# izhengfan/se2lam

Hardware: NVIDIA H100
Metric: ORB keypoints/sec at 640x480 (8-level pyramid, 1000 kps/frame) (higher is better)
Workload: dtype u8

## Files before the change

se2lam_b200/csrc/fast_screen.h:

```cpp
#pragma once
#include <cstdint>

#if defined(__CUDACC__)
#define SE2_HD __host__ __device__ __forceinline__
#else
#define SE2_HD inline
#endif

namespace fastpx {
SE2_HD int16_t lo16(unsigned a) { return (int16_t)(a & 0xFFFF); }
SE2_HD int16_t hi16(unsigned a) { return (int16_t)(a >> 16); }
SE2_HD unsigned pack16(int lo, int hi) { return ((unsigned)lo & 0xFFFFu) | ((unsigned)hi << 16); }
SE2_HD unsigned perm(unsigned a, unsigned b, unsigned s) {
#if defined(__CUDA_ARCH__)
    return __byte_perm(a, b, s);
#else
    const uint64_t src = ((uint64_t)b << 32) | a;
    unsigned r = 0;
    for (int i = 0; i < 4; ++i) {
        const unsigned sel = (s >> (4 * i)) & 0xF;
        unsigned byte = (unsigned)(src >> (8 * (sel & 7))) & 0xFF;
        if (sel & 8) byte = (byte & 0x80) ? 0xFF : 0x00;
        r |= byte << (8 * i);
    }
// ... 38 lines not shown
}

namespace fastpx {

SE2_HD unsigned screen_bias(int t) { return (unsigned)(511 - t) * 0x10001u; }

SE2_HD unsigned screen4(unsigned n3, unsigned s3, unsigned n2l, unsigned n2c, unsigned n2r, unsigned s2l, unsigned s2c, unsigned s2r,
                        unsigned zl, unsigned zc, unsigned zr, unsigned bias) {
    const unsigned w_m3 = perm(zl, zc, 0x4321), w_p3 = perm(zc, zr, 0x6543);
    const unsigned nw_ = perm(n2l, n2c, 0x5432), ne_ = perm(n2c, n2r, 0x5432);
    const unsigned sw_ = perm(s2l, s2c, 0x5432), se_ = perm(s2c, s2r, 0x5432);
    unsigned ok[2];
#if defined(__CUDA_ARCH__)
#pragma unroll
#endif
    for (int hlf = 0; hlf < 2; ++hlf) {
        const unsigned sel = hlf ? 0x4341u : 0x4240u;
        const unsigned v = perm(zc, 0, sel);
        const unsigned p0 = perm(s3, 0, sel), p8 = perm(n3, 0, sel);
        const unsigned p4 = perm(w_p3, 0, sel), p12 = perm(w_m3, 0, sel);
        const unsigned p2 = perm(se_, 0, sel), p10 = perm(nw_, 0, sel);
        const unsigned p6 = perm(ne_, 0, sel), p14 = perm(sw_, 0, sel);
        const unsigned lo = maxs2(max3s2(mins2(p0, p8), mins2(p4, p12), mins2(p2, p10)), mins2(p6, p14));
        const unsigned hi = mins2(min3s2(maxs2(p0, p8), maxs2(p4, p12), maxs2(p2, p10)), maxs2(p6, p14));
        ok[hlf] = ((v + bias - lo) | (hi + bias - v)) & 0x02000200u;
    }
    const unsigned b = ok[0] + (ok[1] << 1);
    return ((b >> 9) | (b >> 23)) & 0xFu;
}
SE2_HD unsigned screen_T1(int t) { return screen_bias(t); }
SE2_HD unsigned screen_U1(int t) { return screen_bias(t); }
SE2_HD unsigned screen4(unsigned n3, unsigned s3, unsigned n2l, unsigned n2c, unsigned n2r, unsigned s2l, unsigned s2c, unsigned s2r,
                        unsigned zl, unsigned zc, unsigned zr, unsigned T1, unsigned ) {
    return screen4(n3, s3, n2l, n2c, n2r, s2l, s2c, s2r, zl, zc, zr, T1);
}

SE2_HD unsigned inside_mask8(int x0, int cw) {
    const int lo = x0 < 0 ? -x0 : 0;
    const int hi = cw - x0 < 8 ? cw - x0 : 8;
    return (0xFFu << lo) & (0xFFu >> (8 - hi)) & 0xFFu;
}

SE2_HD int first_group(int shift) { return (shift + 3) >> 2; }
SE2_HD int groups_per_row(int cw, int shift) { return ((shift + 2 + cw) >> 2) - first_group(shift) + 1; }
SE2_HD int group_x0(int g, int shift) { return 4 * (g + first_group(shift)) - 3 - shift; }
SE2_HD int items_per_row(int cw, int shift) { return (groups_per_row(cw, shift) + 1) >> 1; }
struct ItemWalk {
    int y, g, dY, dG, G;
    SE2_HD void init(int tid, int nthreads, int groups) { G = groups; y = tid / G; g = tid - y * G; dY = nthreads / G; dG = nthreads - dY * G; }
    SE2_HD void next() { g += dG; y += dY; if (g >= G) { g -= G; ++y; } }
};

constexpr int NMS_X0 = 4;
SE2_HD int nms_plane_bytes(int pw, int ch) { return pw * (ch + 2) + 32; }
SE2_HD int nms_words_per_row(int cw) { return (cw + 31) >> 5; }
SE2_HD unsigned nms_row_mask(int k, int cw) { const int n = cw - 32 * k; return n >= 32 ? 0xFFFFFFFFu : (1u << n) - 1u; }

SE2_HD unsigned nms32(const uint32_t* u, const uint32_t* c, const uint32_t* d) {
    unsigned c3e[10], c3o[10];
    unsigned r[4];
#if defined(__CUDA_ARCH__)
#pragma unroll
#endif
    for (int j = 0; j < 10; ++j) {
        const unsigned ua = u[j], ca = c[j], da = d[j];
        if (j > 0) c3e[j] = max3s2(perm(ua, 0, 0x4240), perm(ca, 0, 0x4240), perm(da, 0, 0x4240));
        if (j < 9) c3o[j] = max3s2(perm(ua, 0, 0x4341), perm(ca, 0, 0x4341), perm(da, 0, 0x4341));
    }
#if defined(__CUDA_ARCH__)
#pragma unroll
#endif
    for (int g = 0; g < 8; ++g) {
        const int j = g + 1;
        const unsigned ua = u[j], ca = c[j], da = d[j];
        const unsigned ce = perm(ca, 0, 0x4240), co = perm(ca, 0, 0x4341);
        const unsigned ve = maxs2(perm(ua, 0, 0x4240), perm(da, 0, 0x4240));
        const unsigned vo = maxs2(perm(ua, 0, 0x4341), perm(da, 0, 0x4341));
        const unsigned ne = max3s2(perm(c3o[j - 1], c3o[j], 0x5432), ve, c3o[j]);
        const unsigned no = max3s2(c3e[j], vo, perm(c3e[j], c3e[j + 1], 0x5432));
        const unsigned te = ce + 0x00FF00FFu - ne, to = co + 0x00FF00FFu - no;
        const unsigned bytes = perm(te, to, 0x7351);
        if (g & 1) {
            r[g >> 1] = (r[g >> 1] + (bytes << 4)) * 0x01020408u;
        } else {
            r[g >> 1] = bytes;
        }
    }
    return perm(perm(r[0], r[1], 0x7373), perm(r[2], r[3], 0x7373), 0x5410);
}

struct WordRun {
    int w, w1, y, k, wpr;
    SE2_HD void init(int tid, int nthreads, int ch, int words_per_row) {
        wpr = words_per_row;
        const int nw = ch * wpr, q = (nw + nthreads - 1) / nthreads;
        w = tid * q < nw ? tid * q : nw;
        w1 = w + q < nw ? w + q : nw;
        y = w / wpr; k = w - y * wpr;
    }
    SE2_HD bool more() const { return w < w1; }
    SE2_HD void next() { ++w; if (++k == wpr) { k = 0; ++y; } }
};

}
```

se2lam_b200/csrc/orb.cu:

```cuda
#include <cuda.h>

#include <algorithm>
#include <cmath>
#include <cstring>
#include <type_traits>
#include <vector>

#include "blur_px.h"
#include "common.h"
#include "fast_screen.h"
#include "introselect.h"
#include "resp_key.h"

namespace {

using se2gpu::fail;

constexpr int EDGE = 16;
constexpr int HALF_PATCH = 15;
constexpr int PATCH = 31;
constexpr int MAX_LEVELS = 16;
constexpr int FAST_THREADS = 256;
constexpr int ORB_LANES = 4;
constexpr int BLUR_WARPS = 4;
// ... 247 lines not shown
            for (int r = ty; r < nsr; r += 8) {
                const uint8_t* rp = raw + r * raw_pitch;
                const unsigned h0 = (unsigned)((rp[sx0[0]] * a0[0] + rp[sx1[0]] * a1[0]) >> 4), h1 = (unsigned)((rp[sx0[1]] * a0[1] + rp[sx1[1]] * a1[1]) >> 4);
                const unsigned h2 = (unsigned)((rp[sx0[2]] * a0[2] + rp[sx1[2]] * a1[2]) >> 4), h3 = (unsigned)((rp[sx0[3]] * a0[3] + rp[sx1[3]] * a1[3]) >> 4);
                *reinterpret_cast<uint2*>(hbuf + r * 128 + 4 * tx) = make_uint2((h0 & 0xFFFFu) | (h1 << 16), (h2 & 0xFFFFu) | (h3 << 16));
            }
        }
    }
    __syncthreads();
    if (x4 >= L.pitch) return;
    uint8_t* plane = d.plain + f * d.frame_plane_bytes + L.plane_off;
#pragma unroll
    for (int k = 0; k < RESIZE_TR / 8; ++k) {
        const int r = ty + 8 * k, y = y0 + r;
        if (y >= H) break;
        uint32_t word = 0;
        if (x4 < W) {
            const ResizeRow ri = rowinfo[r];
            const uint2 A = *reinterpret_cast<const uint2*>(hbuf + (ri.s0 - r_lo) * 128 + 4 * tx);
            const uint2 B = *reinterpret_cast<const uint2*>(hbuf + (ri.s1 - r_lo) * 128 + 4 * tx);
            const unsigned v0 = (unsigned)((((ri.b0 * (int)(A.x & 0xFFFFu)) >> 16) + ((ri.b1 * (int)(B.x & 0xFFFFu)) >> 16) + 2) >> 2);
            const unsigned v1 = (unsigned)((((ri.b0 * (int)(A.x >> 16)) >> 16) + ((ri.b1 * (int)(B.x >> 16)) >> 16) + 2) >> 2);
            const unsigned v2 = (unsigned)((((ri.b0 * (int)(A.y & 0xFFFFu)) >> 16) + ((ri.b1 * (int)(B.y & 0xFFFFu)) >> 16) + 2) >> 2);
            const unsigned v3 = (unsigned)((((ri.b0 * (int)(A.y >> 16)) >> 16) + ((ri.b1 * (int)(B.y >> 16)) >> 16) + 2) >> 2);
            word = (v0 | (v1 << 8) | (v2 << 16) | (v3 << 24)) & vmask;
        }
        *reinterpret_cast<uint32_t*>(plane + (size_t)y * L.pitch + x4) = word;
    }
}

__device__ __forceinline__ unsigned fast_cv(int v) { return (unsigned)(256 + v) | ((unsigned)(256 - v) << 16); }
__device__ __forceinline__ unsigned fast_q(unsigned p, unsigned cv) { return p * 0xFFFFu + cv; }

__device__ __forceinline__ int fast_arc_score(const uint8_t* __restrict__ p, int pw) {
    const unsigned cv = fast_cv(p[0]);
    unsigned q[16];
    q[0] = fast_q(p[3 * pw], cv);       q[1] = fast_q(p[3 * pw + 1], cv);   q[2] = fast_q(p[2 * pw + 2], cv);    q[3] = fast_q(p[pw + 3], cv);
    q[4] = fast_q(p[3], cv);            q[5] = fast_q(p[-pw + 3], cv);      q[6] = fast_q(p[-2 * pw + 2], cv);   q[7] = fast_q(p[-3 * pw + 1], cv);
    q[8] = fast_q(p[-3 * pw], cv);      q[9] = fast_q(p[-3 * pw - 1], cv);  q[10] = fast_q(p[-2 * pw - 2], cv);  q[11] = fast_q(p[-pw - 3], cv);
    q[12] = fast_q(p[-3], cv);          q[13] = fast_q(p[pw - 3], cv);      q[14] = fast_q(p[2 * pw - 2], cv);   q[15] = fast_q(p[3 * pw - 1], cv);
    unsigned m3[16];
#pragma unroll
    for (int k = 0; k < 16; ++k) m3[k] = __vimin3_s16x2(q[k], q[(k + 1) & 15], q[(k + 2) & 15]);
    unsigned best = 0;
#pragma unroll
    for (int k = 0; k < 16; k += 2) {
        const unsigned a9 = __vimin3_s16x2(m3[k], m3[(k + 3) & 15], m3[(k + 6) & 15]);
        const unsigned b9 = __vimin3_s16x2(m3[k + 1], m3[(k + 4) & 15], m3[(k + 7) & 15]);
        best = __vimax3_s16x2(best, a9, b9);
    }
    return (int)max(best & 0xFFFFu, best >> 16) - 256;
}

struct FastMaps { CUtensorMap m[MAX_LEVELS]; };
__device__ __forceinline__ unsigned orb_smem_u32(const void* p) { return (unsigned)__cvta_generic_to_shared(p); }
__device__ __forceinline__ void orb_mbar_init(unsigned long long* bar, unsigned count) {
    asm volatile("mbarrier.init.shared::cta.b64 [%0], %1;" ::"r"(orb_smem_u32(bar)), "r"(count) : "memory");
    asm volatile("fence.mbarrier_init.release.cluster;" ::: "memory");
}
__device__ __forceinline__ bool orb_mbar_wait(unsigned long long* bar, unsigned parity) {
    const long long t0 = clock64();
    for (;;) {
        unsigned done;
        asm volatile(
            "{\n"
            ".reg .pred p;\n"
            "mbarrier.try_wait.parity.shared::cta.b64 p, [%1], %2;\n"
            "selp.u32 %0, 1, 0, p;\n"
            "}\n" : "=r"(done) : "r"(orb_smem_u32(bar)), "r"(parity) : "memory");
        if (done) return true;
        if (clock64() - t0 > 400000000LL) return false;
    }
}
__device__ __forceinline__ void orb_tma_box3(void* dst_smem, const CUtensorMap* map, int x, int y, int z, unsigned bytes, unsigned long long* bar) {
    asm volatile("mbarrier.arrive.expect_tx.shared::cta.b64 _, [%0], %1;" ::"r"(orb_smem_u32(bar)), "r"(bytes) : "memory");
    asm volatile("cp.async.bulk.tensor.3d.shared::cluster.global.tile.mbarrier::complete_tx::bytes [%0], [%1, {%2, %3, %4}], [%5];"
                 ::"r"(orb_smem_u32(dst_smem)), "l"(map), "r"(x), "r"(y), "r"(z), "r"(orb_smem_u32(bar)) : "memory");
}

template <bool TMA>
__global__ void __launch_bounds__(FAST_THREADS, 5) orb_fast_cells(OrbDev d, const __grid_constant__ FastMaps maps) {
    extern __shared__ __align__(128) uint8_t smem_raw[];
    __shared__ int s_ncand, s_wsum[FAST_THREADS / 32];
    __shared__ __align__(8) unsigned long long s_bar;
    const CellGeo c = d.cells[blockIdx.x];
    const int f = blockIdx.y + d.frame0;
    CellHdr* hdr = d.hdr + (size_t)f * d.n_cells + blockIdx.x;
    const int cw = c.x1 - c.x0, ch = c.y1 - c.y0;
    if (c.skipped || cw <= 0 || ch <= 0) {
        if (threadIdx.x == 0) { hdr->n_base = 0; hdr->n_a = 0; hdr->n_b = 0; }
        return;
    }
    const LevelGeo& L = d.levels[c.level];
    const int bx0 = c.x0 - 3 + EDGE, ax0 = bx0 & (TMA ? ~15 : ~3), shift = bx0 - ax0;
    const int pw = TMA ? L.fbw : (shift + cw + 6 + 3) & ~3, pww = pw >> 2;
    const int ph = TMA ? L.fbh : ch + 6;
    uint8_t* smem = TMA ? smem_raw + ((128u - (orb_smem_u32(smem_raw) & 127u)) & 127u) : smem_raw;
    const int g0 = fastpx::first_group(shift), G = fastpx::items_per_row(cw, shift), nitems = ch * G;
    const int wpr = fastpx::nms_words_per_row(cw);
    uint8_t* patch = smem;
    uint8_t* score = smem + ((pw * ph + 15) & ~15);
    uint32_t* bitmap = reinterpret_cast<uint32_t*>(score + ((fastpx::nms_plane_bytes(pw, ch) + 15) & ~15));
    uint16_t* list = reinterpret_cast<uint16_t*>(bitmap + ch * wpr);
    if (TMA) {
        if (threadIdx.x == 0) orb_mbar_init(&s_bar, 1);
        __syncthreads();
        if (threadIdx.x == 0) orb_tma_box3(patch, &maps.m[c.level], ax0, c.y0 - 3 + EDGE, f, (unsigned)(pw * ph), &s_bar);
    } else {
        const uint8_t* plane = d.plain + f * d.frame_plane_bytes + L.plane_off;
        const int by0 = c.y0 - 3 + EDGE;
        for (int i = threadIdx.x; i < pww * ph; i += FAST_THREADS) {
            const int py = i / pww, pxw = i - py * pww;
            reinterpret_cast<uint32_t*>(patch)[i] = *reinterpret_cast<const uint32_t*>(plane + (size_t)(by0 + py) * L.pitch + ax0 + 4 * pxw);
        }
    }
    constexpr int NW = FAST_THREADS / 32;
    const int lane = threadIdx.x & 31, wid = threadIdx.x >> 5;
    const uint8_t* p0 = patch + 3 * pw + 3 + shift;
    fastpx::ItemWalk first;
    first.init((int)threadIdx.x, FAST_THREADS, G);
    fastpx::WordRun words;
    words.init((int)threadIdx.x, FAST_THREADS, ch, wpr);
    int thr = d.fast_th;
    int total = 0, pos0 = 0;
    for (int pass = 0; pass < 2; ++pass) {
        for (int i = threadIdx.x; i < pw * (ch + 2) / 4; i += FAST_THREADS) reinterpret_cast<uint32_t*>(score)[i] = 0u;
        if (threadIdx.x == 0) s_ncand = 0;
        if (TMA && pass == 0 && !orb_mbar_wait(&s_bar, 0)) { *d.err = 4; return; }
        __syncthreads();
        {
            const uint32_t* pwords = reinterpret_cast<const uint32_t*>(patch);
            const unsigned bias = fastpx::screen_bias(thr);
            fastpx::ItemWalk it = first;
            for (int it0 = wid * 32; it0 < nitems; it0 += NW * 32) {
                unsigned m = 0;
                const int col0 = fastpx::group_x0(2 * it.g, shift);
                if (it.y < ch) {
                    const uint32_t* c = pwords + (it.y + 3) * pww + 2 * it.g + g0;
                    const uint32_t n3a = c[-3 * pww], n3b = c[-3 * pww + 1], s3a = c[3 * pww], s3b = c[3 * pww + 1];
                    const uint32_t n2a = c[-2 * pww - 1], n2b = c[-2 * pww], n2c = c[-2 * pww + 1], n2d = c[-2 * pww + 2];
                    const uint32_t s2a = c[2 * pww - 1], s2b = c[2 * pww], s2c = c[2 * pww + 1], s2d = c[2 * pww + 2];
                    const uint32_t za = c[-1], zb = c[0], zc = c[1], zd = c[2];
                    m = (fastpx::screen4(n3a, s3a, n2a, n2b, n2c, s2a, s2b, s2c, za, zb, zc, bias) |
                         fastpx::screen4(n3b, s3b, n2b, n2c, n2d, s2b, s2c, s2d, zb, zc, zd, bias) << 4) & fastpx::inside_mask8(col0, cw);
                }
                uint16_t* dst = list + atomicAdd(&s_ncand, __popc(m));
                const int e0 = it.y * pw + col0;
#pragma unroll
                for (int j = 0; j < 8; ++j)
                    if (m & (1u << j)) *dst++ = (uint16_t)(e0 + j);
                it.next();
            }
        }
        __syncthreads();
        const int ncand = s_ncand;
        for (int i = threadIdx.x; i < ncand; i += FAST_THREADS) {
            const int off = list[i];
            const int m = fast_arc_score(p0 + off, pw);
            if (m > thr) score[off + pw + fastpx::NMS_X0] = (uint8_t)(m - 1);
        }
        __syncthreads();
        int nkp = 0;
        for (fastpx::WordRun r = words; r.more(); r.next()) {
            const uint32_t* u = reinterpret_cast<const uint32_t*>(score) + r.y * pww + 8 * r.k;
            const unsigned bits = fastpx::nms32(u, u + pww, u + 2 * pww) & fastpx::nms_row_mask(r.k, cw);
            bitmap[r.w] = bits;
            nkp += __popc(bits);
        }
        int inc = nkp;
#pragma unroll
        for (int o = 1; o < 32; o <<= 1) { const int u = __shfl_up_sync(0xffffffffu, inc, o); if (lane >= o) inc += u; }
        if (lane == 31) s_wsum[wid] = inc;
        __syncthreads();
        total = 0; pos0 = inc - nkp;
#pragma unroll
        for (int w = 0; w < NW; ++w) { const int v = s_wsum[w]; total += v; if (w < wid) pos0 += v; }
        if (total > 3 || thr == 7) break;
        thr = 7;
    }
    uint32_t* out = d.cand + (size_t)f * d.cand_total + c.cand_off;
    int pos = pos0;
    for (fastpx::WordRun r = words; r.more(); r.next()) {
        uint32_t bits = bitmap[r.w];
        const uint8_t* srow = score + (r.y + 1) * pw + fastpx::NMS_X0 + 32 * r.k;
        const uint32_t yx = ((uint32_t)(c.y0 + r.y) << 12) | (uint32_t)(c.x0 + 32 * r.k);
        while (bits) {
            const int i = __ffs(bits) - 1;
            bits &= bits - 1;
            if (pos < c.cand_cap) out[pos] = ((uint32_t)srow[i] << 24) | (yx + i);
            else *d.err = 1;
            ++pos;
        }
    }
    if (threadIdx.x == 0) { hdr->n_base = total; hdr->n_a = total; hdr->n_b = total; }
}

__device__ __forceinline__ int fast_arc_score_qr(const uint8_t* __restrict__ p, int pw, int t) {
    const int v = p[0];
    const int c0 = v - p[3 * pw], c8 = v - p[-3 * pw];
    bool dk = (c0 > t) | (c8 > t), br = (c0 < -t) | (c8 < -t);
    if (!(dk | br)) return 0;
    const int c4 = v - p[3], c12 = v - p[-3];
    dk &= (c4 > t) | (c12 > t); br &= (c4 < -t) | (c12 < -t);
    if (!(dk | br)) return 0;
    const int c2 = v - p[2 * pw + 2], c10 = v - p[-2 * pw - 2];
    dk &= (c2 > t) | (c10 > t); br &= (c2 < -t) | (c10 < -t);
    if (!(dk | br)) return 0;
    const int c6 = v - p[-2 * pw + 2], c14 = v - p[2 * pw - 2];
    dk &= (c6 > t) | (c14 > t); br &= (c6 < -t) | (c14 < -t);
    if (!(dk | br)) return 0;
#define SE2_PK(dv) ((static_cast<unsigned>(dv) & 0xFFFFu) | (static_cast<unsigned>(-(dv)) << 16))
    unsigned q[16];
    q[0] = SE2_PK(c0);   q[1] = SE2_PK(v - p[3 * pw + 1]);    q[2] = SE2_PK(c2);    q[3] = SE2_PK(v - p[pw + 3]);
    q[4] = SE2_PK(c4);   q[5] = SE2_PK(v - p[-pw + 3]);       q[6] = SE2_PK(c6);    q[7] = SE2_PK(v - p[-3 * pw + 1]);
    q[8] = SE2_PK(c8);   q[9] = SE2_PK(v - p[-3 * pw - 1]);   q[10] = SE2_PK(c10);  q[11] = SE2_PK(v - p[-pw - 3]);
    q[12] = SE2_PK(c12); q[13] = SE2_PK(v - p[pw - 3]);       q[14] = SE2_PK(c14);  q[15] = SE2_PK(v - p[3 * pw - 1]);
#undef SE2_PK
    unsigned m3[16];
#pragma unroll
    for (int k = 0; k < 16; ++k) m3[k] = __vimin3_s16x2(q[k], q[(k + 1) & 15], q[(k + 2) & 15]);
    unsigned best = 0x80008000u;
#pragma unroll
    for (int k = 0; k < 16; k += 2) {
        const unsigned a9 = __vimin3_s16x2(m3[k], m3[(k + 3) & 15], m3[(k + 6) & 15]);
        const unsigned b9 = __vimin3_s16x2(m3[k + 1], m3[(k + 4) & 15], m3[(k + 7) & 15]);
        best = __vimax3_s16x2(best, a9, b9);
    }
    const int mdark = static_cast<short>(best & 0xFFFFu), mbright = static_cast<short>(best >> 16);
    return max(mdark, mbright);
}

__global__ void __launch_bounds__(FAST_THREADS) orb_fast_cells_big(OrbDev d) {
    extern __shared__ uint8_t smem[];
    __shared__ int s_total;
    const CellGeo c = d.cells[blockIdx.x];
    const int f = blockIdx.y + d.frame0;
    CellHdr* hdr = d.hdr + (size_t)f * d.n_cells + blockIdx.x;
    const int cw = c.x1 - c.x0, ch = c.y1 - c.y0;
    if (c.skipped || cw <= 0 || ch <= 0) {
        if (threadIdx.x == 0) { hdr->n_base = 0; hdr->n_a = 0; hdr->n_b = 0; }
        return;
    }
    const LevelGeo& L = d.levels[c.level];
    const uint8_t* plane = d.plain + f * d.frame_plane_bytes + L.plane_off;
    const int bx0 = c.x0 - 3 + EDGE, by0 = c.y0 - 3 + EDGE;
    const int ax0 = bx0 & ~3, shift = bx0 - ax0;
    const int ph = ch + 6, sw = cw + 2, sh = ch + 2;
// ... 486 lines not shown
    int kp_off = 0;
    const float imageRatio = (float)w / (float)hgt;
    for (int l = 0; l < nl; ++l) {
        LevelGeo& g = L[l];
        const float scale = h->mvInvScaleFactor[l];
        g.w = cv_round_f((float)w * scale); g.h = cv_round_f((float)hgt * scale);
        if (g.w < 2 * EDGE + 7 || g.h < 2 * EDGE + 7) return fail(SE2GPU_ERR_INVALID, "level %d of a %dx%d frame is %dx%d: too small for the 16 px border", l, w, hgt, g.w, g.h);
        if (g.w + 2 * EDGE > 4095 || g.h + 2 * EDGE > 4095) return fail(SE2GPU_ERR_CAPACITY, "frames wider/taller than 4063 px are not supported");
        g.pitch = (g.w + 2 * EDGE + 31) & ~31;
        g.plane_off = poff;
        poff += (size_t)g.pitch * (g.h + 2 * EDGE);
        poff = (poff + 255) & ~(size_t)255;
        g.nDesired = h->mnFeaturesPerLevel[l];
        g.cols = (int)sqrtf((float)g.nDesired / (5 * imageRatio));
        g.rows = (int)(imageRatio * g.cols);
        if (g.cols < 1 || g.rows < 1) return fail(SE2GPU_ERR_INVALID, "level %d has a %dx%d cell grid (nfeatures too small): undefined in the reference", l, g.cols, g.rows);
        const int minB = EDGE, maxBX = g.w - EDGE, maxBY = g.h - EDGE;
        const int W = maxBX - minB, H = maxBY - minB;
        const int cellW = (int)ceilf((float)W / g.cols), cellH = (int)ceilf((float)H / g.rows);
        g.nCells = g.rows * g.cols;
        g.nfeaturesCell = (int)ceilf((float)g.nDesired / g.nCells);
        g.cell_base = (int)C.size();
        g.kp_off = kp_off; g.kp_cap = g.nDesired; kp_off += g.nDesired;
        g.scale = h->mvScaleFactor[l];
        g.kp_size = (float)(int)(PATCH * h->mvScaleFactor[l]);
        g.tab_off = (int)toff; toff += (size_t)g.w + g.h;
        std::vector<int> iniXCol(g.cols, 0);
        const size_t first_cell = C.size();
        int max_cw = 0, max_ch = 0;
        float hY = cellH + 6;
        for (int i = 0; i < g.rows; ++i) {
            const float iniY = minB + i * cellH - 3;
            bool rowSkipped = false;
            if (i == g.rows - 1) { hY = maxBY + 3 - iniY; if (hY <= 0) rowSkipped = true; }
            float hX = cellW + 6;
            for (int j = 0; j < g.cols; ++j) {
                CellGeo c{};
                c.level = l;
                if (rowSkipped) { c.skipped = 1; C.push_back(c); continue; }
                float iniX;
                if (i == 0) { iniX = minB + j * cellW - 3; iniXCol[j] = (int)iniX; } else iniX = iniXCol[j];
                if (j == g.cols - 1) { hX = maxBX + 3 - iniX; if (hX <= 0) { c.skipped = 1; C.push_back(c); continue; } }
                const int r0 = (int)iniY, r1 = (int)(iniY + hY), c0 = (int)iniX, c1 = (int)(iniX + hX);
                if (r1 > g.h || c1 > g.w || r0 < 0 || c0 < 0) return fail(SE2GPU_ERR_INVALID, "cell grid of level %d leaves the image (the reference asserts here)", l);
                c.x0 = c0 + 3; c.x1 = c1 - 3; c.y0 = r0 + 3; c.y1 = r1 - 3;
                const int cw = std::max(c.x1 - c.x0, 0), chh = std::max(c.y1 - c.y0, 0);
                c.cand_off = (int)coff;
                c.cand_cap = ((cw + 1) / 2) * ((chh + 1) / 2) + 8;
                coff += c.cand_cap;
                if (cw > 0 && chh > 0) {
                    max_cw = std::max(max_cw, ((c.x0 - 3 + EDGE) & 15) + cw); max_ch = std::max(max_ch, chh);
                    const size_t pwb = (size_t)((cw + 6 + 3 + 3) / 4 + 1) * 4;
                    const size_t bitmap = (size_t)chh * fastpx::nms_words_per_row(cw) * 4;
                    if (pwb * (chh + 6) > 65535) fast_big = true;
                    fsm = std::max(fsm, ((pwb * (chh + 6) + 15) & ~(size_t)15) + (((size_t)fastpx::nms_plane_bytes((int)pwb, chh) + 15) & ~(size_t)15) + bitmap + (size_t)cw * chh * 2 + 64);
                    const size_t nchunk = (size_t)chh * ((cw + 31) / 32);
                    fsm_big = std::max(fsm_big, ((pwb * (chh + 6) + 15) & ~(size_t)15) + (((size_t)(cw + 2) * (chh + 2) + 15) & ~(size_t)15) + nchunk * 4 + 64);
                }
                C.push_back(c);
            }
        }
        g.fbw = (max_cw + 6 + 15) & ~15; g.fbh = max_ch + 6;
        if (max_cw > 0) {
            if (g.fbw > 256 || g.fbh > 256 || (size_t)g.fbw * g.fbh > 65535) tma_ok = false;
            for (size_t ci = first_cell; ci < C.size(); ++ci) {
                const int cw = C[ci].x1 - C[ci].x0, chh = C[ci].y1 - C[ci].y0;
                if (C[ci].skipped || cw <= 0 || chh <= 0) continue;
                const size_t pw = (size_t)g.fbw, bitmap = (size_t)chh * fastpx::nms_words_per_row(cw) * 4;
                fsm_tma = std::max(fsm_tma, (size_t)128 + ((pw * g.fbh + 15) & ~(size_t)15) + (((size_t)fastpx::nms_plane_bytes(g.fbw, chh) + 15) & ~(size_t)15) + bitmap + (size_t)cw * chh * 2 + 64);
            }
        }
        if (h->harris) ssm = std::max(ssm, (size_t)(2 * g.nDesired + 4 * g.nCells + 64) * 8 + (size_t)g.nCells * 16 + (size_t)(SEL_STAGE / 2) * 8);
        else ssm = std::max(ssm, (size_t)(2 * g.nDesired + 4 * g.nCells + 64) * 4 + (size_t)g.nCells * 16 + (size_t)SEL_STAGE * 4);
        g.tile_base = (int)T.size();
        g.blur_strips = std::max(2, (g.h + BLUR_TH - 1) / BLUR_TH);
        g.blur_th = ((g.h + g.blur_strips - 1) / g.blur_strips + 12) / 7 * 7 - 6;
        for (int it = 0; it < g.blur_strips * (g.pitch / 8); it += 32) T.push_back(TileGeo{l, it / (g.pitch / 8), it % (g.pitch / 8)});
    }
    *plane_bytes = poff; *cand_total = coff; *n_cells = C.size(); *n_tiles = T.size(); *tab_total = toff;
    if (fsm > 227 * 1024) fast_big = true;
    *max_fast_smem = fast_big ? fsm_big : fsm; *max_select_smem = ssm;
    if (fast_big_out) *fast_big_out = fast_big;
    if (fast_tma_smem_out) *fast_tma_smem_out = (tma_ok && !fast_big && fsm_tma <= 227 * 1024) ? fsm_tma : 0;
    if (Lv) *Lv = L;
    if (Cv) *Cv = C;
    if (Tv) *Tv = T;
    return SE2GPU_OK;
}

typedef CUresult (*EncodeTiledFn)(CUtensorMap*, CUtensorMapDataType, cuuint32_t, void*, const cuuint64_t*, const cuuint64_t*, const cuuint32_t*,
                                  const cuuint32_t*, CUtensorMapInterleave, CUtensorMapSwizzle, CUtensorMapL2promotion, CUtensorMapFloatOOBfill);
EncodeTiledFn tensor_map_encoder() {
    static EncodeTiledFn fn = [] {
        void* p = nullptr;
        cudaDriverEntryPointQueryResult q = cudaDriverEntryPointSymbolNotFound;
        if (cudaGetDriverEntryPoint("cuTensorMapEncodeTiled", &p, cudaEnableDefault, &q) != cudaSuccess || q != cudaDriverEntryPointSuccess) { cudaGetLastError(); p = nullptr; }
        return (EncodeTiledFn)p;
    }();
    return fn;
}

constexpr int BLUR_SPLIT = 1;
constexpr int PIPE_CHUNKS = 4, PIPE_FIRST_PCT = 50, SUBMIT_CHUNKS = 1;

bool encode_fast_maps(se2gpu_orb* h, size_t frame_plane_bytes) {
    EncodeTiledFn enc = tensor_map_encoder();
    if (!enc || (frame_plane_bytes & 15)) return false;
    for (int l = 0; l < h->nlevels; ++l) {
        const LevelGeo& g = h->levels[l];
        if (g.fbw <= 6) { memset(&h->fast_maps.m[l], 0, sizeof(CUtensorMap)); continue; }
        const cuuint64_t gdim[3] = {(cuuint64_t)g.pitch, (cuuint64_t)(g.h + 2 * EDGE), (cuuint64_t)h->max_batch};
        const cuuint64_t gstr[2] = {(cuuint64_t)g.pitch, (cuuint64_t)frame_plane_bytes};
        const cuuint32_t box[3] = {(cuuint32_t)g.fbw, (cuuint32_t)g.fbh, 1u};
        const cuuint32_t estr[3] = {1u, 1u, 1u};
        void* base = h->d.plain + g.plane_off;
        if (((uintptr_t)base & 15) || (g.pitch & 15)) return false;
        if (enc(&h->fast_maps.m[l], CU_TENSOR_MAP_DATA_TYPE_UINT8, 3, base, gdim, gstr, box, estr, CU_TENSOR_MAP_INTERLEAVE_NONE,
                CU_TENSOR_MAP_SWIZZLE_NONE, CU_TENSOR_MAP_L2_PROMOTION_L2_128B, CU_TENSOR_MAP_FLOAT_OOB_FILL_NONE) != CUDA_SUCCESS) return false;
    }
    return true;
}

int set_geometry(se2gpu_orb* h, int w, int hgt, cudaStream_t s) {
    if (w == h->cur_w && hgt == h->cur_h) return SE2GPU_OK;
    size_t pb, ct, nc, nt, tt, fsm, ssm, fsm_tma = 0;
    bool big = false;
    int rc = build_geometry(h, w, hgt, false, &pb, &ct, &nc, &nt, &tt, &fsm, &ssm, &h->levels, &h->cells, &h->tiles, &big, &fsm_tma);
    if (rc != SE2GPU_OK) return rc;
    if (pb > h->cap_plane || ct > h->cap_cand || nc > h->cap_cells || nt > h->cap_tiles || tt > h->cap_tab)
        return fail(SE2GPU_ERR_CAPACITY, "frame %dx%d exceeds the capacity this extractor was created with (%dx%d)", w, hgt, h->max_w, h->max_h);
    if (fsm > 227 * 1024) return fail(SE2GPU_ERR_CAPACITY, "a FAST cell of a %dx%d frame needs %zu B of shared memory", w, hgt, fsm);
    std::vector<int> itab(tt, 0);
    std::vector<short> stab(2 * tt, 0);
    for (int l = 1; l < h->nlevels; ++l) {
        const LevelGeo& g = h->levels[l];
        const LevelGeo& sg = h->levels[l - 1];
        const double scale_x = 1. / ((double)g.w / sg.w), scale_y = 1. / ((double)g.h / sg.h);
        int* xofs = itab.data() + g.tab_off; int* yofs = xofs + g.w;
        short* ialpha = stab.data() + 2 * (size_t)g.tab_off; short* ibeta = ialpha + 2 * g.w;
        for (int dx = 0; dx < g.w; ++dx) {
            float fx = (float)((dx + 0.5) * scale_x - 0.5);
            int sx = (int)floorf(fx);
            fx -= sx;
            if (sx < 0) { fx = 0; sx = 0; }
            if (sx >= sg.w - 1) { fx = 0; sx = sg.w - 1; }
            xofs[dx] = sx;
            ialpha[2 * dx] = (short)std::min(std::max(cv_round_f((1.f - fx) * 2048.f), -32768), 32767);
            ialpha[2 * dx + 1] = (short)std::min(std::max(cv_round_f(fx * 2048.f), -32768), 32767);
        }
        for (int dy = 0; dy < g.h; ++dy) {
            float fy = (float)((dy + 0.5) * scale_y - 0.5);
            int sy = (int)floorf(fy);
            fy -= sy;
            yofs[dy] = sy;
            ibeta[2 * dy] = (short)cv_round_f((1.f - fy) * 2048.f);
            ibeta[2 * dy + 1] = (short)cv_round_f(fy * 2048.f);
        }
    }
    SE2_CUDA(cudaMemcpyAsync(h->d_levels, h->levels.data(), sizeof(LevelGeo) * h->levels.size(), cudaMemcpyHostToDevice, s));
    SE2_CUDA(cudaMemcpyAsync(h->d_cells, h->cells.data(), sizeof(CellGeo) * h->cells.size(), cudaMemcpyHostToDevice, s));
    SE2_CUDA(cudaMemcpyAsync(h->d_tiles, h->tiles.data(), sizeof(TileGeo) * h->tiles.size(), cudaMemcpyHostToDevice, s));
    SE2_CUDA(cudaMemcpyAsync(h->d_itab, itab.data(), sizeof(int) * itab.size(), cudaMemcpyHostToDevice, s));
// ... 117 lines not shown
    d.frame0 = frame0;
    cudaStream_t side = lane < 0 ? h->side : nullptr;
    cudaEvent_t ev_pyr = h->ev_pyr, ev_blur = h->ev_blur;
    se2gpu::Profiler& pr = h->prof;
    SE2_NVTX("se2gpu.orb.run_device");
    nvtxRangePushA("se2gpu.orb.pyramid");
    pr.begin(0, s);
    {
        const LevelGeo& g = h->levels[0];
        if (h->und_on) {
            dim3 grid((g.pitch / 4 + 127) / 128, g.h + 2 * EDGE, n);
            SE2_LAUNCH(orb_pyr0_undistort, grid, 128, 0, s, d, g, d_imgs, stride, frame_stride, h->d_und_m1, h->d_und_m2);
        } else {
            const int aligned = (((uintptr_t)d_imgs | (uintptr_t)stride | (uintptr_t)frame_stride) & 15) == 0;
            const int nvec = aligned ? g.w / 16 : 0;
            dim3 grid((nvec + 63) / 64 + 1, (g.h + 2 * EDGE + 4 * PYR0_ROWS - 1) / (4 * PYR0_ROWS), n);
            SE2_LAUNCH(orb_pyr0, grid, dim3(64, 4), 0, s, d, g, d_imgs, stride, frame_stride, nvec);
        }
    }
    const int splitA = std::min(BLUR_SPLIT, h->nlevels);
    for (int l = 1; l < h->nlevels; ++l) {
        const LevelGeo& g = h->levels[l];
        cudaLaunchConfig_t cfg = {};
        const int ncx = (g.pitch + 127) / 128, H = g.h + 2 * EDGE;
        const int tall_grid = ncx * ((H + RESIZE_TR_TALL - 1) / RESIZE_TR_TALL) * n;
        const bool tall = h->resize_tall_ctas > 0 && tall_grid >= h->resize_tall_ctas;
        const int tr = tall ? RESIZE_TR_TALL : RESIZE_TR;
        cfg.gridDim = dim3(ncx, (H + tr - 1) / tr, n);
        cfg.blockDim = dim3(32, 8); cfg.dynamicSmemBytes = tall ? h->resize_tall_smem : h->resize_w_smem; cfg.stream = s;
        cudaLaunchAttribute at[1];
        at[0].id = cudaLaunchAttributeProgrammaticStreamSerialization;
        at[0].val.programmaticStreamSerializationAllowed = 1;
        cfg.attrs = at; cfg.numAttrs = 1;
        if (tall) SE2_CUDA(cudaLaunchKernelEx(&cfg, orb_resize_w<RESIZE_TR_TALL>, d, g, h->levels[l - 1], h->resize_tall_rows, h->resize_raw_pitch));
        else SE2_CUDA(cudaLaunchKernelEx(&cfg, orb_resize_w<RESIZE_TR>, d, g, h->levels[l - 1], h->resize_rows, h->resize_raw_pitch));
        ::se2gpu::g_launches.fetch_add(1, std::memory_order_relaxed);
        if (l == splitA - 1 && side && !pr.on) SE2_CUDA(cudaEventRecord(h->ev_l1, s));
    }
    if (splitA - 1 <= 0 && side && !pr.on) SE2_CUDA(cudaEventRecord(h->ev_l1, s));
    pr.end(s);
    nvtxRangePop();
    const bool overlap = !pr.on && side != nullptr;
    auto launch_blur = [&](cudaStream_t st, int t0, int t1) {
        if (t1 > t0) SE2_LAUNCH(orb_blur, dim3((t1 - t0 + BLUR_WARPS - 1) / BLUR_WARPS, n), BLUR_WARPS * 32, 0, st, d, t0, t1);
    };
    const int tilesA = splitA < h->nlevels ? h->levels[splitA].tile_base : d.n_tiles;
    if (overlap) {
        SE2_CUDA(cudaStreamWaitEvent(side, h->ev_l1, 0));
        launch_blur(side, 0, tilesA);
    }
    SE2_NVTX("se2gpu.orb.fast_select_blur_describe");
    pr.begin(1, s);
    if (h->fast_big) SE2_LAUNCH(orb_fast_cells_big, dim3(d.n_cells, n), FAST_THREADS, h->fast_smem, s, d);
    else if (h->fast_tma) SE2_LAUNCH(orb_fast_cells<true>, dim3(d.n_cells, n), FAST_THREADS, h->fast_tma_smem, s, d, h->fast_maps);
    else SE2_LAUNCH(orb_fast_cells<false>, dim3(d.n_cells, n), FAST_THREADS, h->fast_smem, s, d, h->fast_maps);
    if (h->harris) SE2_LAUNCH(orb_harris, dim3(d.n_cells, n), HARRIS_THREADS, 0, s, d, h->hb.cand64);
    pr.end(s);
    if (overlap) {
        SE2_CUDA(cudaEventRecord(ev_pyr, s));
        SE2_CUDA(cudaStreamWaitEvent(side, ev_pyr, 0));
        launch_blur(side, tilesA, d.n_tiles);
        SE2_CUDA(cudaEventRecord(ev_blur, side));
    }
    pr.begin(2, s);
    if (h->harris) SE2_LAUNCH(orb_select<true>, dim3(h->nlevels, n), SEL_THREADS, h->select_smem, s, d, h->hb);
    else SE2_LAUNCH(orb_select<false>, dim3(h->nlevels, n), SEL_THREADS, h->select_smem, s, d, h->hb);
    pr.end(s);
    if (overlap) {
        SE2_CUDA(cudaStreamWaitEvent(s, ev_blur, 0));
    } else {
        pr.begin(3, s);
        launch_blur(s, 0, d.n_tiles);
        pr.end(s);
    }
    const int warps = 8;
    pr.begin(4, s);
    if (h->harris) SE2_LAUNCH(orb_orient_describe<true>, dim3((h->nfeatures + warps - 1) / warps, n), warps * 32, 0, s, d, d_kps, d_desc, d_counts, h->hb.lresp);
    else SE2_LAUNCH(orb_orient_describe<false>, dim3((h->nfeatures + warps - 1) / warps, n), warps * 32, 0, s, d, d_kps, d_desc, d_counts, h->hb.lresp);
    pr.end(s);
    h->last_n = std::max(h->last_n * (frame0 > 0), frame0 + n);
    return SE2GPU_OK;
}

}

extern "C" {

se2gpu_orb* se2gpu_orb_create_scored(int nfeatures, float scale_factor, int nlevels, int score_type, int fast_th, int max_w, int max_h,
                                     int max_batch, int device) {
    if (score_type != SE2GPU_ORB_HARRIS_SCORE && score_type != SE2GPU_ORB_FAST_SCORE) {
        fail(SE2GPU_ERR_INVALID, "unknown ORB score type %d (HARRIS_SCORE = 0, FAST_SCORE = 1)", score_type); return nullptr;
    }
    if (nfeatures <= 0 || nlevels <= 0 || nlevels > MAX_LEVELS || !(scale_factor > 1.0f) || fast_th < 1 || fast_th > 254 ||
        max_w <= 0 || max_h <= 0 || max_batch <= 0) { fail(SE2GPU_ERR_INVALID, "bad ORB parameters"); return nullptr; }
    if (se2gpu::select_device(device) != SE2GPU_OK) return nullptr;
    se2gpu_orb* h = new se2gpu_orb;
    h->device = device; h->nfeatures = nfeatures; h->nlevels = nlevels; h->fast_th = fast_th;
    h->harris = score_type == SE2GPU_ORB_HARRIS_SCORE;
    h->max_w = max_w; h->max_h = max_h; h->max_batch = max_batch;
    { int* a = h->create_args; a[0] = nfeatures; memcpy(&a[1], &scale_factor, sizeof(float)); a[2] = nlevels; a[3] = fast_th; a[4] = max_w; a[5] = max_h; a[6] = max_batch; a[7] = device; a[8] = score_type; }
    h->scaleFactor = scale_factor;
    h->mvScaleFactor.resize(nlevels); h->mvInvScaleFactor.resize(nlevels); h->mnFeaturesPerLevel.resize(nlevels);
    h->mvScaleFactor[0] = 1;
    for (int i = 1; i < nlevels; i++) h->mvScaleFactor[i] = (float)(h->mvScaleFactor[i - 1] * h->scaleFactor);
    const float invScaleFactor = (float)(1.0f / h->scaleFactor);
    h->mvInvScaleFactor[0] = 1;
    for (int i = 1; i < nlevels; i++) h->mvInvScaleFactor[i] = h->mvInvScaleFactor[i - 1] * invScaleFactor;
    const float factor = (float)(1.0 / h->scaleFactor);
// ... 243 lines not shown
int se2gpu_orb_set_undistort(se2gpu_orb* h, const float* K, const float* dist, int ndist) {
    if (!h) return fail(SE2GPU_ERR_INVALID, "null handle");
    if (!K) { h->und_on = false; return SE2GPU_OK; }
    if (ndist != 0 && ndist != 4 && ndist != 5 && ndist != 8 && ndist != 12 && ndist != 14) return fail(SE2GPU_ERR_INVALID, "distortion vector must have 0, 4, 5, 8, 12 or 14 coefficients");
    if (ndist > 0 && !dist) return fail(SE2GPU_ERR_INVALID, "null distortion vector");
    if (ndist == 14 && (dist[12] != 0.f || dist[13] != 0.f)) return fail(SE2GPU_ERR_INVALID, "tilted-sensor coefficients (tauX, tauY) are not supported");
    memcpy(h->und_K, K, sizeof h->und_K);
    memset(h->und_D, 0, sizeof h->und_D);
    if (ndist > 0) memcpy(h->und_D, dist, sizeof(float) * ndist);
    h->und_nd = ndist; h->und_w = h->und_h = 0; h->und_on = true;
    return SE2GPU_OK;
}

int se2gpu_orb_debug_undistort_map(const float* K, const float* dist, int ndist, int w, int hgt, int16_t* m1, uint16_t* m2) {
    if (!K || !m1 || !m2 || w <= 0 || hgt <= 0 || ndist < 0 || ndist > 14 || (ndist > 0 && !dist)) return fail(SE2GPU_ERR_INVALID, "bad argument");
    std::vector<short2> a; std::vector<uint16_t> b;
    int rc = build_undistort_map(K, dist, ndist, w, hgt, a, b);
    if (rc != SE2GPU_OK) return rc;
    memcpy(m1, a.data(), a.size() * sizeof(short2));
    memcpy(m2, b.data(), b.size() * sizeof(uint16_t));
    return SE2GPU_OK;
}

int se2gpu_orb_profile(se2gpu_orb* h, int enable) {
    if (!h) return fail(SE2GPU_ERR_INVALID, "null handle");
    SE2_CUDA(cudaSetDevice(h->device));
    h->prof.enable(enable != 0);
    return SE2GPU_OK;
}

int se2gpu_orb_profile_read(se2gpu_orb* h, double* ms, int* launches) {
    if (!h) return fail(SE2GPU_ERR_INVALID, "null handle");
    SE2_CUDA(cudaSetDevice(h->device));
    h->prof.flush();
    for (int g = 0; g < SE2GPU_ORB_PROFILE_GROUPS; ++g) { if (ms) ms[g] = h->prof.ms[g]; if (launches) launches[g] = h->prof.launches[g]; }
    return SE2GPU_OK;
}

int se2gpu_orb_level_dims(se2gpu_orb* h, int level, int* w, int* hgt, int* pitch) {
    if (!h || level < 0 || level >= h->nlevels || h->cur_w < 0) return fail(SE2GPU_ERR_INVALID, "no geometry");
    *w = h->levels[level].w; *hgt = h->levels[level].h; *pitch = h->levels[level].pitch;
    return SE2GPU_OK;
}

int se2gpu_orb_get_level(se2gpu_orb* h, int frame, int level, int blurred, uint8_t* out) {
    if (!h || level < 0 || level >= h->nlevels || h->cur_w < 0 || frame < 0 || frame >= h->last_n) return fail(SE2GPU_ERR_INVALID, "bad frame/level");
    SE2_CUDA(cudaSetDevice(h->device));
    const LevelGeo& g = h->levels[level];
    const uint8_t* src = (blurred ? h->d.blurred : h->d.plain) + (size_t)frame * h->d.frame_plane_bytes + g.plane_off;
    SE2_CUDA(cudaMemcpy(out, src, (size_t)g.pitch * (g.h + 2 * EDGE), cudaMemcpyDeviceToHost));
    return SE2GPU_OK;
}

}
```

Measured before the change: 109.6 million.

## Pad NMS score pitch, flatten FAST grid cell-major, pass box dims in maps

The NMS score plane now uses a separate pitch (pw | 4), which skews rows to reduce shared-memory bank conflicts in the 3-row nms32 reads. The TMA path adds a per-row skew via a reciprocal multiply to map patch offsets to the padded score layout. The FAST launch is flattened to a 1D grid, ordered cell-major with frames interleaved, so blocks for the same cell across frames run adjacently. Box dimensions now come from the grid-constant FastMaps instead of the global level struct. Optional clock instrumentation is added behind a compile flag. The padding uses slightly more shared memory per block, which may affect occupancy.

New measurement: 112.2 million, median of 6. +2.4%, better.

```diff
diff --git a/se2lam_b200/csrc/fast_screen.h b/se2lam_b200/csrc/fast_screen.h
--- a/se2lam_b200/csrc/fast_screen.h
+++ b/se2lam_b200/csrc/fast_screen.h
@@ -114,7 +114,8 @@
 };
 
 constexpr int NMS_X0 = 4;
-SE2_HD int nms_plane_bytes(int pw, int ch) { return pw * (ch + 2) + 32; }
+SE2_HD int nms_pitch(int pw) { return pw | 4; }
+SE2_HD int nms_plane_bytes(int sp, int ch) { return sp * (ch + 2) + 32; }
 SE2_HD int nms_words_per_row(int cw) { return (cw + 31) >> 5; }
 SE2_HD unsigned nms_row_mask(int k, int cw) { const int n = cw - 32 * k; return n >= 32 ? 0xFFFFFFFFu : (1u << n) - 1u; }
 
diff --git a/se2lam_b200/csrc/orb.cu b/se2lam_b200/csrc/orb.cu
--- a/se2lam_b200/csrc/orb.cu
+++ b/se2lam_b200/csrc/orb.cu
@@ -323,7 +323,7 @@
     return (int)max(best & 0xFFFFu, best >> 16) - 256;
 }
 
-struct FastMaps { CUtensorMap m[MAX_LEVELS]; };
+struct FastMaps { CUtensorMap m[MAX_LEVELS]; int fbw[MAX_LEVELS], fbh[MAX_LEVELS]; };
 __device__ __forceinline__ unsigned orb_smem_u32(const void* p) { return (unsigned)__cvta_generic_to_shared(p); }
 __device__ __forceinline__ void orb_mbar_init(unsigned long long* bar, unsigned count) {
     asm volatile("mbarrier.init.shared::cta.b64 [%0], %1;" ::"r"(orb_smem_u32(bar)), "r"(count) : "memory");
@@ -349,34 +349,56 @@
                  ::"r"(orb_smem_u32(dst_smem)), "l"(map), "r"(x), "r"(y), "r"(z), "r"(orb_smem_u32(bar)) : "memory");
 }
 
+#ifdef SE2GPU_FAST_PASS_CLOCKS
+enum FastClk { CLK_ENTRY = 0, CLK_LANDED = 1, CLK_PASS0 = 2,  CLK_END = 8,
+               CLK_INFO = 9 , CLK_GT0 = 10, CLK_GT1 = 11, CLK_ISSUED = 12 ,
+               FAST_CLK_SLOTS = 13 };
+__device__ unsigned long long* g_fast_clk;
+__device__ __forceinline__ unsigned long long orb_globaltimer() { unsigned long long t; asm volatile("mov.u64 %0, %%globaltimer;" : "=l"(t)); return t; }
+__device__ __forceinline__ unsigned orb_smid() { unsigned s; asm volatile("mov.u32 %0, %%smid;" : "=r"(s)); return s; }
+#define FAST_CLK(slot, v) do { if (threadIdx.x == 0 && g_fast_clk) g_fast_clk[((size_t)f * d.n_cells + cell) * FAST_CLK_SLOTS + (slot)] = (v); } while (0)
+#else
+#define FAST_CLK(slot, v) do { } while (0)
+#endif
+
 template <bool TMA>
 __global__ void __launch_bounds__(FAST_THREADS, 5) orb_fast_cells(OrbDev d, const __grid_constant__ FastMaps maps) {
     extern __shared__ __align__(128) uint8_t smem_raw[];
     __shared__ int s_ncand, s_wsum[FAST_THREADS / 32];
     __shared__ __align__(8) unsigned long long s_bar;
-    const CellGeo c = d.cells[blockIdx.x];
-    const int f = blockIdx.y + d.frame0;
-    CellHdr* hdr = d.hdr + (size_t)f * d.n_cells + blockIdx.x;
+    const int frames = gridDim.x / d.n_cells, cell = blockIdx.x / frames;
+    const CellGeo c = d.cells[cell];
+    const int f = blockIdx.x - cell * frames + d.frame0;
+    CellHdr* hdr = d.hdr + (size_t)f * d.n_cells + cell;
     const int cw = c.x1 - c.x0, ch = c.y1 - c.y0;
+#ifdef SE2GPU_FAST_PASS_CLOCKS
+    FAST_CLK(CLK_GT0, orb_globaltimer());
+    FAST_CLK(CLK_ENTRY, clock64());
+    FAST_CLK(CLK_INFO, (unsigned long long)(c.level | orb_smid() << 16));
+#endif
     if (c.skipped || cw <= 0 || ch <= 0) {
         if (threadIdx.x == 0) { hdr->n_base = 0; hdr->n_a = 0; hdr->n_b = 0; }
         return;
     }
     const LevelGeo& L = d.levels[c.level];
     const int bx0 = c.x0 - 3 + EDGE, ax0 = bx0 & (TMA ? ~15 : ~3), shift = bx0 - ax0;
-    const int pw = TMA ? L.fbw : (shift + cw + 6 + 3) & ~3, pww = pw >> 2;
-    const int ph = TMA ? L.fbh : ch + 6;
+    const int pw = TMA ? maps.fbw[c.level] : fastpx::nms_pitch((shift + cw + 6 + 3) & ~3), pww = pw >> 2;
+    const int ph = TMA ? maps.fbh[c.level] : ch + 6;
     uint8_t* smem = TMA ? smem_raw + ((128u - (orb_smem_u32(smem_raw) & 127u)) & 127u) : smem_raw;
     const int g0 = fastpx::first_group(shift), G = fastpx::items_per_row(cw, shift), nitems = ch * G;
     const int wpr = fastpx::nms_words_per_row(cw);
+    const int sp = fastpx::nms_pitch(pw), spw = sp >> 2;
     uint8_t* patch = smem;
     uint8_t* score = smem + ((pw * ph + 15) & ~15);
-    uint32_t* bitmap = reinterpret_cast<uint32_t*>(score + ((fastpx::nms_plane_bytes(pw, ch) + 15) & ~15));
+    uint32_t* bitmap = reinterpret_cast<uint32_t*>(score + ((fastpx::nms_plane_bytes(sp, ch) + 15) & ~15));
     uint16_t* list = reinterpret_cast<uint16_t*>(bitmap + ch * wpr);
     if (TMA) {
         if (threadIdx.x == 0) orb_mbar_init(&s_bar, 1);
         __syncthreads();
         if (threadIdx.x == 0) orb_tma_box3(patch, &maps.m[c.level], ax0, c.y0 - 3 + EDGE, f, (unsigned)(pw * ph), &s_bar);
+#ifdef SE2GPU_FAST_PASS_CLOCKS
+        FAST_CLK(CLK_ISSUED, clock64());
+#endif
     } else {
         const uint8_t* plane = d.plain + f * d.frame_plane_bytes + L.plane_off;
         const int by0 = c.y0 - 3 + EDGE;
@@ -395,9 +417,10 @@
     int thr = d.fast_th;
     int total = 0, pos0 = 0;
     for (int pass = 0; pass < 2; ++pass) {
-        for (int i = threadIdx.x; i < pw * (ch + 2) / 4; i += FAST_THREADS) reinterpret_cast<uint32_t*>(score)[i] = 0u;
+        for (int i = threadIdx.x; i < spw * (ch + 2); i += FAST_THREADS) reinterpret_cast<uint32_t*>(score)[i] = 0u;
         if (threadIdx.x == 0) s_ncand = 0;
         if (TMA && pass == 0 && !orb_mbar_wait(&s_bar, 0)) { *d.err = 4; return; }
+        if (pass == 0) FAST_CLK(CLK_LANDED, clock64());
         __syncthreads();
         {
             const uint32_t* pwords = reinterpret_cast<const uint32_t*>(patch);
@@ -424,17 +447,23 @@
             }
         }
         __syncthreads();
+        FAST_CLK(CLK_PASS0 + 3 * pass, clock64());
         const int ncand = s_ncand;
-        for (int i = threadIdx.x; i < ncand; i += FAST_THREADS) {
-            const int off = list[i];
-            const int m = fast_arc_score(p0 + off, pw);
-            if (m > thr) score[off + pw + fastpx::NMS_X0] = (uint8_t)(m - 1);
+        {
+            const unsigned rpw = 0xFFFFFFFFu / (unsigned)pw + 1u;
+            for (int i = threadIdx.x; i < ncand; i += FAST_THREADS) {
+                const int off = list[i];
+                const int m = fast_arc_score(p0 + off, pw);
+                const int skew = TMA ? 4 * (int)__umulhi((unsigned)off, rpw) : 0;
+                if (m > thr) score[off + skew + sp + fastpx::NMS_X0] = (uint8_t)(m - 1);
+            }
         }
         __syncthreads();
+        FAST_CLK(CLK_PASS0 + 3 * pass + 1, clock64());
         int nkp = 0;
         for (fastpx::WordRun r = words; r.more(); r.next()) {
-            const uint32_t* u = reinterpret_cast<const uint32_t*>(score) + r.y * pww + 8 * r.k;
-            const unsigned bits = fastpx::nms32(u, u + pww, u + 2 * pww) & fastpx::nms_row_mask(r.k, cw);
+            const uint32_t* u = reinterpret_cast<const uint32_t*>(score) + r.y * spw + 8 * r.k;
+            const unsigned bits = fastpx::nms32(u, u + spw, u + 2 * spw) & fastpx::nms_row_mask(r.k, cw);
             bitmap[r.w] = bits;
             nkp += __popc(bits);
         }
@@ -446,6 +475,10 @@
         total = 0; pos0 = inc - nkp;
 #pragma unroll
         for (int w = 0; w < NW; ++w) { const int v = s_wsum[w]; total += v; if (w < wid) pos0 += v; }
+        FAST_CLK(CLK_PASS0 + 3 * pass + 2, clock64());
+#ifdef SE2GPU_FAST_PASS_CLOCKS
+        FAST_CLK(CLK_INFO, (unsigned long long)(c.level | (pass + 1) << 8 | orb_smid() << 16));
+#endif
         if (total > 3 || thr == 7) break;
         thr = 7;
     }
@@ -453,7 +486,7 @@
     int pos = pos0;
     for (fastpx::WordRun r = words; r.more(); r.next()) {
         uint32_t bits = bitmap[r.w];
-        const uint8_t* srow = score + (r.y + 1) * pw + fastpx::NMS_X0 + 32 * r.k;
+        const uint8_t* srow = score + (r.y + 1) * sp + fastpx::NMS_X0 + 32 * r.k;
         const uint32_t yx = ((uint32_t)(c.y0 + r.y) << 12) | (uint32_t)(c.x0 + 32 * r.k);
         while (bits) {
             const int i = __ffs(bits) - 1;
@@ -464,6 +497,11 @@
         }
     }
     if (threadIdx.x == 0) { hdr->n_base = total; hdr->n_a = total; hdr->n_b = total; }
+#ifdef SE2GPU_FAST_PASS_CLOCKS
+    __syncthreads();
+    FAST_CLK(CLK_END, clock64());
+    FAST_CLK(CLK_GT1, orb_globaltimer());
+#endif
 }
 
 __device__ __forceinline__ int fast_arc_score_qr(const uint8_t* __restrict__ p, int pw, int t) {
@@ -1056,8 +1094,9 @@
                     max_cw = std::max(max_cw, ((c.x0 - 3 + EDGE) & 15) + cw); max_ch = std::max(max_ch, chh);
                     const size_t pwb = (size_t)((cw + 6 + 3 + 3) / 4 + 1) * 4;
                     const size_t bitmap = (size_t)chh * fastpx::nms_words_per_row(cw) * 4;
-                    if (pwb * (chh + 6) > 65535) fast_big = true;
-                    fsm = std::max(fsm, ((pwb * (chh + 6) + 15) & ~(size_t)15) + (((size_t)fastpx::nms_plane_bytes((int)pwb, chh) + 15) & ~(size_t)15) + bitmap + (size_t)cw * chh * 2 + 64);
+                    const size_t ppw = (size_t)fastpx::nms_pitch((int)pwb);
+                    if (ppw * (chh + 6) > 65535) fast_big = true;
+                    fsm = std::max(fsm, ((ppw * (chh + 6) + 15) & ~(size_t)15) + (((size_t)fastpx::nms_plane_bytes((int)ppw, chh) + 15) & ~(size_t)15) + bitmap + (size_t)cw * chh * 2 + 64);
                     const size_t nchunk = (size_t)chh * ((cw + 31) / 32);
                     fsm_big = std::max(fsm_big, ((pwb * (chh + 6) + 15) & ~(size_t)15) + (((size_t)(cw + 2) * (chh + 2) + 15) & ~(size_t)15) + nchunk * 4 + 64);
                 }
@@ -1071,7 +1110,7 @@
                 const int cw = C[ci].x1 - C[ci].x0, chh = C[ci].y1 - C[ci].y0;
                 if (C[ci].skipped || cw <= 0 || chh <= 0) continue;
                 const size_t pw = (size_t)g.fbw, bitmap = (size_t)chh * fastpx::nms_words_per_row(cw) * 4;
-                fsm_tma = std::max(fsm_tma, (size_t)128 + ((pw * g.fbh + 15) & ~(size_t)15) + (((size_t)fastpx::nms_plane_bytes(g.fbw, chh) + 15) & ~(size_t)15) + bitmap + (size_t)cw * chh * 2 + 64);
+                fsm_tma = std::max(fsm_tma, (size_t)128 + ((pw * g.fbh + 15) & ~(size_t)15) + (((size_t)fastpx::nms_plane_bytes(fastpx::nms_pitch(g.fbw), chh) + 15) & ~(size_t)15) + bitmap + (size_t)cw * chh * 2 + 64);
             }
         }
         if (h->harris) ssm = std::max(ssm, (size_t)(2 * g.nDesired + 4 * g.nCells + 64) * 8 + (size_t)g.nCells * 16 + (size_t)(SEL_STAGE / 2) * 8);
@@ -1112,6 +1151,7 @@
     if (!enc || (frame_plane_bytes & 15)) return false;
     for (int l = 0; l < h->nlevels; ++l) {
         const LevelGeo& g = h->levels[l];
+        h->fast_maps.fbw[l] = g.fbw; h->fast_maps.fbh[l] = g.fbh;
         if (g.fbw <= 6) { memset(&h->fast_maps.m[l], 0, sizeof(CUtensorMap)); continue; }
         const cuuint64_t gdim[3] = {(cuuint64_t)g.pitch, (cuuint64_t)(g.h + 2 * EDGE), (cuuint64_t)h->max_batch};
         const cuuint64_t gstr[2] = {(cuuint64_t)g.pitch, (cuuint64_t)frame_plane_bytes};
@@ -1335,8 +1375,8 @@
     SE2_NVTX("se2gpu.orb.fast_select_blur_describe");
     pr.begin(1, s);
     if (h->fast_big) SE2_LAUNCH(orb_fast_cells_big, dim3(d.n_cells, n), FAST_THREADS, h->fast_smem, s, d);
-    else if (h->fast_tma) SE2_LAUNCH(orb_fast_cells<true>, dim3(d.n_cells, n), FAST_THREADS, h->fast_tma_smem, s, d, h->fast_maps);
-    else SE2_LAUNCH(orb_fast_cells<false>, dim3(d.n_cells, n), FAST_THREADS, h->fast_smem, s, d, h->fast_maps);
+    else if (h->fast_tma) SE2_LAUNCH(orb_fast_cells<true>, dim3(d.n_cells * n), FAST_THREADS, h->fast_tma_smem, s, d, h->fast_maps);
+    else SE2_LAUNCH(orb_fast_cells<false>, dim3(d.n_cells * n), FAST_THREADS, h->fast_smem, s, d, h->fast_maps);
     if (h->harris) SE2_LAUNCH(orb_harris, dim3(d.n_cells, n), HARRIS_THREADS, 0, s, d, h->hb.cand64);
     pr.end(s);
     if (overlap) {
@@ -1686,4 +1726,14 @@
     return SE2GPU_OK;
 }
 
-}
+#ifdef SE2GPU_FAST_PASS_CLOCKS
+int se2gpu_orb_fast_pass_clocks(se2gpu_orb* h, void* buf, int* n_cells, int* slots) {
+    if (!h || h->cur_w < 0) return fail(SE2GPU_ERR_INVALID, "no geometry");
+    SE2_CUDA(cudaSetDevice(h->device));
+    SE2_CUDA(cudaMemcpyToSymbol(g_fast_clk, &buf, sizeof(buf)));
+    *n_cells = h->d.n_cells; *slots = FAST_CLK_SLOTS;
+    return SE2GPU_OK;
+}
+#endif
+
+}
```
